# RandallBalestriero/noise-robust-vit

Hardware: AMD Instinct MI355X
Metric: images/sec (fwd+bwd+optimizer) ViT-B/16 224px bf16 (higher is better)
Workload: dtype bf16

## Files before the change

noise_robust_vit_amd/csrc/nrv_attn.hip:

```cpp
#include <type_traits>

#include "nrv_attn_common.hpp"

NRV_INTERNAL int nrv_attn_gen_supported(int B, int N, int H, int dh);
NRV_INTERNAL int nrv_attn_gen_fwd(const void* qkv, void* out, float* lse, int B, int N, int H, int dh, float scale, hipStream_t s);
NRV_INTERNAL int nrv_attn_gen_bwd(const void* qkv, const void* out, const void* dout, const float* lse, void* dqkv, float* delta_ws,
                     int B, int N, int H, int dh, float scale, hipStream_t s);
NRV_INTERNAL int nrv_attn_gen_probs(const void* qkv, const float* lse, float* probs, int B, int N, int H, int dh, float scale, hipStream_t s);

namespace {

using namespace nrv_attn;
struct AttnParams {
    const bf16_t* qkv;
    const bf16_t* out;
    const bf16_t* dout;
    bf16_t* o;
    bf16_t* dqkv;
    float* lse;
    float* delta;
    int B, N, H;
    float scale;
    long long q_rs, q_ws, q_hs, q_bs, o_rs, o_hs, o_bs;
};

void set_layout(AttnParams& p, int layout, int dh) {
    const long long T = (long long)p.B * p.N;
    if (layout & NRV_ATTN_QKV_BLOCKED) { p.q_rs = dh; p.q_ws = (long long)p.H * T * dh; p.q_hs = T * dh; p.q_bs = (long long)p.N * dh; }
    else { p.q_rs = 3ll * p.H * dh; p.q_ws = (long long)p.H * dh; p.q_hs = dh; p.q_bs = p.N * p.q_rs; }
    if (layout & NRV_ATTN_OUT_BLOCKED) { p.o_rs = dh; p.o_hs = T * dh; p.o_bs = (long long)p.N * dh; }
    else { p.o_rs = (long long)p.H * dh; p.o_hs = dh; p.o_bs = p.N * p.o_rs; }
}

template <int NT>
constexpr int atf_waves() { return NT <= 2 ? 1 : NT <= 4 ? 2 : 4; }

template <int NT>
__global__ __launch_bounds__(64 * atf_waves<NT>(), NT <= 13 ? 3 : 2) void attn_fwd_fat_kernel(const AttnParams p) {
    extern __shared__ __attribute__((aligned(16))) char smem[];
    constexpr int NP = NT * 16;
    constexpr int IMG = NP * 128;
    constexpr int NS = (NT + 1) / 2;
    constexpr int NJ = 2 * NP / 8;
    constexpr int ATF_WAVES = atf_waves<NT>();
    constexpr int JPW = NJ / ATF_WAVES;
    constexpr int MT = (NT == 13 || NT == 14) ? 1 : 2;
    const int tid = threadIdx.x, lane = tid & 63, wave = tid >> 6;
    const int N = p.N, H = p.H;
    const long long ldq = p.q_rs;
    const int b = blockIdx.x / H, h = blockIdx.x - b * H;
    const bf16_t* hb = p.qkv + (long long)b * p.q_bs + h * p.q_hs;
    const int g = lane >> 4, qc = lane & 15;
    const float sc = p.scale * LOG2E;
    const char* kimg = smem;
    const char* vimg = smem + IMG;

    const int npairs = (N + 31) >> 5;
    bf16x8_t qf[2][2];
    auto load_q = [&](int pair) {
#pragma unroll
        for (int t = 0; t < 2; ++t) {
            const int q = pair * 32 + t * 16 + qc;
            const int qr = q < N ? q : N - 1;
#pragma unroll
            for (int ks = 0; ks < 2; ++ks) qf[t][ks] = load_frag_global(hb + (long long)qr * ldq + ks * 32 + g * 8);
        }
    };
    if (wave < npairs) load_q(wave);
    {
        const __amdgpu_buffer_rsrc_t rk = make_rsrc(hb + p.q_ws, 0x7fffffffull), rv = make_rsrc(hb + 2 * p.q_ws, 0x7fffffffull);
        const int wave_u = __builtin_amdgcn_readfirstlane(wave);
#pragma unroll
        for (int i = 0; i < JPW; ++i) {
            const int j = wave_u * JPW + i;
            const bool isv = j >= NP / 8;
            const int r = 8 * (isv ? j - NP / 8 : j) + (lane >> 3);
            const int pos = lane & 7;
            const int c = isv ? ((((pos >> 1) ^ ((r >> 1) & 3)) << 1) | (pos & 1)) : (pos ^ ((r >> 1) & 7));
            const unsigned vo = (r < N) ? (unsigned)(r * ldq * 2 + c * 16) : NRV_OOB;
            if (isv) dma16_nt(rv, smem + j * 1024, vo);
            else dma16_nt(rk, smem + j * 1024, vo);
        }
    }
    __builtin_amdgcn_s_waitcnt(0x0F70);
    asm volatile("" ::: "memory");
    __syncthreads();

    const bf16x4_t zero4 = {0, 0, 0, 0};
    auto v_frag = [&](int kk, int dt) {
        const int q = (lane & 15) >> 2, pp = lane & 3;
        const int r0 = kk * 32 + 4 * g + q;
        const bf16x4_t lo = lds_read_tr16_b64(vimg + r0 * 128 + ((dt ^ ((r0 >> 1) & 3)) << 5) + pp * 8);
        if (2 * kk + 1 >= NT) return cat4(lo, zero4);
        return cat4(lo, lds_read_tr16_b64(vimg + (r0 + 16) * 128 + ((dt ^ (((r0 + 16) >> 1) & 3)) << 5) + pp * 8));
    };
    const int d_lane = (g & 1) ? 16 + 4 * (g - 1) : 4 * g;
    for (int pair = wave; pair < npairs; pair += ATF_WAVES) {
        f32x4_t st[2][NT];
        constexpr int KD = NT < 4 ? NT : 4;
        bf16x8_t kf[KD][2];
#pragma unroll
        for (int j = 0; j < KD - 1; ++j)
#pragma unroll
            for (int ks = 0; ks < 2; ++ks) kf[j][ks] = row_frag_img(kimg, j * 16, ks, lane);
#pragma unroll
        for (int kt = 0; kt < NT; ++kt) {
            if (kt + KD - 1 < NT) {
#pragma unroll
                for (int ks = 0; ks < 2; ++ks) kf[(kt + KD - 1) % KD][ks] = row_frag_img(kimg, (kt + KD - 1) * 16, ks, lane);
            }
#pragma unroll
            for (int t = 0; t < 2; ++t) {
                f32x4_t a = {0.f, 0.f, 0.f, 0.f};
#pragma unroll
                for (int ks = 0; ks < 2; ++ks) a = mfma16(kf[kt % KD][ks], qf[t][ks], a);
                st[t][kt] = a;
            }
        }
        __builtin_amdgcn_sched_barrier(0);
        const int q0 = pair * 32 + qc;
        if (pair + ATF_WAVES < npairs) load_q(pair + ATF_WAVES);
        bf16x8_t vf[2][4];
#pragma unroll
        for (int dt = 0; dt < 4; ++dt) vf[0][dt] = v_frag(0, dt);
        float m[2], l[2];
        bf16x8_t pf[2][NS];
#pragma unroll
        for (int t = 0; t < 2; ++t) {
            float mm = -INFINITY;
#pragma unroll
            for (int kt = 0; kt < NT; ++kt) {
#pragma unroll
                for (int e = 0; e < 4; ++e) {
                    if (kt >= NT - MT) mm = fmaxf(mm, (kt * 16 + 4 * g + e < N) ? st[t][kt][e] : -INFINITY);
                    else mm = fmaxf(mm, st[t][kt][e]);
                }
            }
            mm = fmaxf(mm, __shfl_xor(mm, 16, 64));
            mm = fmaxf(mm, __shfl_xor(mm, 32, 64));
            mm *= sc;
            float ll = 0.f;
#pragma unroll
            for (int kt = 0; kt < NT; ++kt) {
#pragma unroll
                for (int e = 0; e < 4; ++e) {
                    float pv = __builtin_amdgcn_exp2f(fmaf(st[t][kt][e], sc, -mm));
                    if (kt >= NT - MT) pv = (kt * 16 + 4 * g + e < N) ? pv : 0.f;
                    st[t][kt][e] = pv;
                    ll += pv;
                }
                if (kt & 1) pf[t][kt >> 1] = pack_frag(st[t][kt - 1], st[t][kt]);
                else if (kt == NT - 1) pf[t][kt >> 1] = pack_frag(st[t][kt], f32x4_t{0.f, 0.f, 0.f, 0.f});
            }
            ll += __shfl_xor(ll, 16, 64);
            ll += __shfl_xor(ll, 32, 64);
            m[t] = mm;
            l[t] = ll;
        }
        __builtin_amdgcn_sched_barrier(0);
        f32x4_t o[2][4];
#pragma unroll
        for (int t = 0; t < 2; ++t)
#pragma unroll
            for (int dt = 0; dt < 4; ++dt) o[t][dt] = f32x4_t{0.f, 0.f, 0.f, 0.f};
#pragma unroll
        for (int kk = 0; kk < NS; ++kk) {
            if (kk + 1 < NS) {
#pragma unroll
                for (int dt = 0; dt < 4; ++dt) vf[(kk + 1) & 1][dt] = v_frag(kk + 1, dt);
            }
#pragma unroll
            for (int dt = 0; dt < 4; ++dt)
#pragma unroll
                for (int t = 0; t < 2; ++t) o[t][dt] = mfma16(vf[kk & 1][dt], pf[t][kk], o[t][dt]);
        }
        __builtin_amdgcn_sched_barrier(0);
#pragma unroll
        for (int t = 0; t < 2; ++t) {
            const int q = q0 + t * 16;
            const float inv = 1.0f / l[t];
            u32x4_t ov[2];
#pragma unroll
            for (int pr = 0; pr < 2; ++pr) {
                const f32x4_t oa = o[t][2 * pr] * inv, ob = o[t][2 * pr + 1] * inv;
                const auto lo = __builtin_amdgcn_permlane16_swap(pack_bf16x2(oa[0], oa[1]), pack_bf16x2(ob[0], ob[1]), false, false);
                const auto hi = __builtin_amdgcn_permlane16_swap(pack_bf16x2(oa[2], oa[3]), pack_bf16x2(ob[2], ob[3]), false, false);
                ov[pr] = u32x4_t{lo[0], hi[0], lo[1], hi[1]};
            }
            if (q < N) {
                bf16_t* dst = p.o + (long long)b * p.o_bs + h * p.o_hs + (long long)q * p.o_rs + d_lane;
#pragma unroll
                for (int pr = 0; pr < 2; ++pr) *reinterpret_cast<u32x4_t*>(dst + 32 * pr) = ov[pr];
                if (g == 0) p.lse[((long long)b * H + h) * N + q] = (m[t] + __builtin_amdgcn_logf(l[t])) * LN2;
            }
        }
    }
}

__device__ __forceinline__ bf16x8_t row_frag_bwd(const char* img, int rb, int ks, int lane) {
    return lds_read_b128(img + vimg_off(rb + (lane & 15), ks * 4 + (lane >> 4)));
}

__device__ __forceinline__ void store_tile_bf16(bf16_t* row_ptr , const f32x4_t (&acc)[4],
                                                float mul, int g, bool ok) {
    const int d_lane = (g & 1) ? 16 + 4 * (g - 1) : 4 * g;
#pragma unroll
    for (int pr = 0; pr < 2; ++pr) {
        const f32x4_t a = acc[2 * pr] * mul, b = acc[2 * pr + 1] * mul;
        const auto lo = __builtin_amdgcn_permlane16_swap(pack_bf16x2(a[0], a[1]), pack_bf16x2(b[0], b[1]), false, false);
        const auto hi = __builtin_amdgcn_permlane16_swap(pack_bf16x2(a[2], a[3]), pack_bf16x2(b[2], b[3]), false, false);
        if (ok) *reinterpret_cast<u32x4_t*>(row_ptr + 32 * pr + d_lane) = u32x4_t{lo[0], hi[0], lo[1], hi[1]};
    }
}

template <int NT>
__device__ __forceinline__ void dma_two_images(char* smem, const bf16_t* src0, long long ld0, const bf16_t* src1, long long ld1,
                                               int N, int wave, int lane) {
    constexpr int NP = NT * 16;
    constexpr int PW = 4 * NT / atf_waves<NT>();
    const __amdgpu_buffer_rsrc_t r0 = make_rsrc(src0, 0x7fffffffull), r1 = make_rsrc(src1, 0x7fffffffull);
    const int wave_u = __builtin_amdgcn_readfirstlane(wave);
#pragma unroll
    for (int i = 0; i < PW; ++i) {
        const int j = wave_u * PW + i;
        const bool second = j >= NP / 8;
        const int r = 8 * (second ? j - NP / 8 : j) + (lane >> 3);
        const int pos = lane & 7;
        const int c = (((pos >> 1) ^ ((r >> 1) & 3)) << 1) | (pos & 1);
        const unsigned vo = (r < N) ? (unsigned)(r * (second ? ld1 : ld0) * 2 + c * 16) : NRV_OOB;
        if (second) dma16(r1, smem + j * 1024, vo);
        else dma16(r0, smem + j * 1024, vo);
    }
}

template <int NT>
__global__ __launch_bounds__(64 * atf_waves<NT>(), NT <= 13 ? 3 : 2) void attn_bwd_dq_fat_kernel(const AttnParams p) {
    extern __shared__ __attribute__((aligned(16))) char smem[];
    constexpr int ATF_WAVES = atf_waves<NT>();
    constexpr int NP = NT * 16;
    constexpr int NS = (NT + 1) / 2;
    constexpr int MT = (NT == 13 || NT == 14) ? 1 : 2;
    const char* kimg = smem;
    const char* vimg = smem + NP * 128;
    const int tid = threadIdx.x, lane = tid & 63, wave = tid >> 6;
    const int N = p.N, H = p.H;
    const int b = blockIdx.x / H, h = blockIdx.x - b * H;
    const long long ldq = p.q_rs, ldo = p.o_rs;
    const bf16_t* qbase = p.qkv + (long long)b * p.q_bs + h * p.q_hs;
    const bf16_t* obase = p.out + (long long)b * p.o_bs + h * p.o_hs;
    const bf16_t* dobase = p.dout + (long long)b * p.o_bs + h * p.o_hs;
    const int g = lane >> 4, qc = lane & 15;
    const float sc = p.scale * LOG2E;
    const int npairs = (N + 31) >> 5;

    bf16x8_t qf[2][2], dof[2][2];
    float dl[2], lse2[2];
    auto load_rows = [&](int pair) {
#pragma unroll
        for (int t = 0; t < 2; ++t) {
            const int q = pair * 32 + t * 16 + qc;
            const int qr = q < N ? q : N - 1;
            float d = 0.f;
#pragma unroll
            for (int ks = 0; ks < 2; ++ks) {
                qf[t][ks] = load_frag_global(qbase + (long long)qr * ldq + ks * 32 + g * 8);
                dof[t][ks] = load_frag_global(dobase + (long long)qr * ldo + ks * 32 + g * 8);
                const bf16x8_t of = load_frag_global(obase + (long long)qr * ldo + ks * 32 + g * 8);
#pragma unroll
                for (int e = 0; e < 8; ++e) d += bf16_to_f32((unsigned short)dof[t][ks][e]) * bf16_to_f32((unsigned short)of[e]);
            }
            d += __shfl_xor(d, 16, 64);
            d += __shfl_xor(d, 32, 64);
            dl[t] = d;
            const long long sidx = ((long long)b * H + h) * N + qr;
            lse2[t] = p.lse[sidx] * LOG2E;
            if (g == 0 && q < N) p.delta[sidx] = d;
        }
    };
    if (wave < npairs) load_rows(wave);
    dma_two_images<NT>(smem, qbase + p.q_ws, ldq, qbase + 2 * p.q_ws, ldq, N, wave, lane);
    __builtin_amdgcn_s_waitcnt(0x0F70);
    asm volatile("" ::: "memory");
    __syncthreads();

    const bf16x4_t zero4 = {0, 0, 0, 0};
    for (int pair = wave; pair < npairs; pair += ATF_WAVES) {
        f32x4_t dq[2][4];
#pragma unroll
        for (int t = 0; t < 2; ++t)
#pragma unroll
            for (int dt = 0; dt < 4; ++dt) dq[t][dt] = f32x4_t{0.f, 0.f, 0.f, 0.f};
        auto step = [&](const int kk, auto last_c) {
            constexpr bool LAST = decltype(last_c)::value;
            f32x4_t ds[2][2];
#pragma unroll
            for (int hf = 0; hf < 2; ++hf) {
                const int kt = 2 * kk + hf;
                if (!LAST || hf == 0 || (NT % 2 == 0)) {
                    bf16x8_t kr[2], vr[2];
#pragma unroll
                    for (int ks = 0; ks < 2; ++ks) {
                        kr[ks] = row_frag_bwd(kimg, kt * 16, ks, lane);
                        vr[ks] = row_frag_bwd(vimg, kt * 16, ks, lane);
                    }
#pragma unroll
                    for (int t = 0; t < 2; ++t) {
                        f32x4_t st = {0.f, 0.f, 0.f, 0.f}, dp = {0.f, 0.f, 0.f, 0.f};
#pragma unroll
                        for (int ks = 0; ks < 2; ++ks) {
                            st = mfma16(kr[ks], qf[t][ks], st);
                            dp = mfma16(vr[ks], dof[t][ks], dp);
                        }
#pragma unroll
                        for (int e = 0; e < 4; ++e) {
                            float pv = __builtin_amdgcn_exp2f(fmaf(st[e], sc, -lse2[t]));
                            if (LAST) pv = (kt * 16 + 4 * g + e < N) ? pv : 0.f;
                            ds[t][hf][e] = pv * (dp[e] - dl[t]);
                        }
                    }
                } else {
#pragma unroll
                    for (int t = 0; t < 2; ++t) ds[t][hf] = f32x4_t{0.f, 0.f, 0.f, 0.f};
                }
            }
            bf16x8_t dsf[2];
#pragma unroll
            for (int t = 0; t < 2; ++t) dsf[t] = pack_frag(ds[t][0], ds[t][1]);
#pragma unroll
            for (int dt = 0; dt < 4; ++dt) {
                const int q4 = (lane & 15) >> 2, pp = lane & 3;
                const int r0 = kk * 32 + 4 * g + q4;
                const int c = 2 * dt + (pp >> 1);
                const bf16x4_t lo = lds_read_tr16_b64(kimg + vimg_off(r0, c) + (pp & 1) * 8);
                const bf16x4_t hi = (!LAST || NT % 2 == 0) ? lds_read_tr16_b64(kimg + vimg_off(r0 + 16, c) + (pp & 1) * 8) : zero4;
                const bf16x8_t ktr = cat4(lo, hi);
#pragma unroll
                for (int t = 0; t < 2; ++t) dq[t][dt] = mfma16(ktr, dsf[t], dq[t][dt]);
            }
        };
#pragma unroll 1
        for (int kk = 0; kk < NS - 1; ++kk) step(kk, std::false_type{});
        step(NS - 1, std::true_type{});
        const int q0 = pair * 32 + qc;
        f32x4_t keep[2][4];
#pragma unroll
        for (int t = 0; t < 2; ++t)
#pragma unroll
            for (int dt = 0; dt < 4; ++dt) keep[t][dt] = dq[t][dt];
        if (pair + ATF_WAVES < npairs) load_rows(pair + ATF_WAVES);
#pragma unroll
        for (int t = 0; t < 2; ++t) {
            const int q = q0 + t * 16;
            store_tile_bf16(p.dqkv + (long long)b * p.q_bs + h * p.q_hs + (long long)(q < N ? q : 0) * ldq, keep[t], p.scale, g, q < N);
        }
    }
}

template <int NT>
__global__ __launch_bounds__(64 * atf_waves<NT>(), 2) void attn_bwd_dkv_fat_kernel(const AttnParams p) {
    extern __shared__ __attribute__((aligned(16))) char smem[];
    constexpr int ATF_WAVES = atf_waves<NT>(), ATF_THREADS = 64 * ATF_WAVES;
    constexpr int NP = NT * 16;
    constexpr int NS = (NT + 1) / 2;
    constexpr int NPS = NS * 32;
    const char* qimg = smem;
    const char* doimg = smem + NP * 128;
    float* lse2s = reinterpret_cast<float*>(smem + 2 * NP * 128);
    float* dels = lse2s + NPS;
    const int tid = threadIdx.x, lane = tid & 63, wave = tid >> 6;
    const int N = p.N, H = p.H;
    const int b = blockIdx.x / H, h = blockIdx.x - b * H;
    const long long ldq = p.q_rs, ldo = p.o_rs;
    const bf16_t* qbase = p.qkv + (long long)b * p.q_bs + h * p.q_hs;
    const bf16_t* dobase = p.dout + (long long)b * p.o_bs + h * p.o_hs;
    const int g = lane >> 4, kc = lane & 15;
    const float sc = p.scale * LOG2E;
    const int npairs = (N + 31) >> 5;

    bf16x8_t kf[2][2], vf[2][2];
    auto load_rows = [&](int pair) {
#pragma unroll
        for (int t = 0; t < 2; ++t) {
            const int key = pair * 32 + t * 16 + kc;
            const int kr = key < N ? key : N - 1;
#pragma unroll
            for (int ks = 0; ks < 2; ++ks) {
                kf[t][ks] = load_frag_global(qbase + p.q_ws + (long long)kr * ldq + ks * 32 + g * 8);
                vf[t][ks] = load_frag_global(qbase + 2 * p.q_ws + (long long)kr * ldq + ks * 32 + g * 8);
            }
        }
    };
    if (wave < npairs) load_rows(wave);
    for (int i = tid; i < NPS; i += ATF_THREADS) {
        const long long sidx = ((long long)b * H + h) * N + i;
        lse2s[i] = i < N ? p.lse[sidx] * LOG2E : INFINITY;
        dels[i] = i < N ? p.delta[sidx] : 0.f;
    }
    dma_two_images<NT>(smem, qbase, ldq, dobase, ldo, N, wave, lane);
    __builtin_amdgcn_s_waitcnt(0x0F70);
    asm volatile("" ::: "memory");
    __syncthreads();

    const bf16x4_t zero4 = {0, 0, 0, 0};
    auto tr_frag = [&](const char* img, int qq, int dt, auto last_c) {
        const int q4 = (lane & 15) >> 2, pp = lane & 3;
        const int r0 = qq * 32 + 4 * g + q4;
        const int c = 2 * dt + (pp >> 1);
        const bf16x4_t lo = lds_read_tr16_b64(img + vimg_off(r0, c) + (pp & 1) * 8);
        const bf16x4_t hi = (!decltype(last_c)::value || NT % 2 == 0) ? lds_read_tr16_b64(img + vimg_off(r0 + 16, c) + (pp & 1) * 8) : zero4;
        return cat4(lo, hi);
    };
    for (int pair = wave; pair < npairs; pair += ATF_WAVES) {
        f32x4_t dk[2][4], dv[2][4];
#pragma unroll
        for (int t = 0; t < 2; ++t)
#pragma unroll
            for (int dt = 0; dt < 4; ++dt) {
                dk[t][dt] = f32x4_t{0.f, 0.f, 0.f, 0.f};
                dv[t][dt] = dk[t][dt];
            }
        auto step = [&](const int qq, auto last_c) {
            constexpr bool LAST = decltype(last_c)::value;
            f32x4_t pt[2][2], ds[2][2];
#pragma unroll
            for (int hf = 0; hf < 2; ++hf) {
                const int qt = 2 * qq + hf;
                if (!LAST || hf == 0 || (NT % 2 == 0)) {
                    bf16x8_t qr[2], dor[2];
#pragma unroll
                    for (int ks = 0; ks < 2; ++ks) {
                        qr[ks] = row_frag_bwd(qimg, qt * 16, ks, lane);
                        dor[ks] = row_frag_bwd(doimg, qt * 16, ks, lane);
                    }
                    const f32x4_t l4 = *reinterpret_cast<const f32x4_t*>(lse2s + qt * 16 + 4 * g);
                    const f32x4_t d4 = *reinterpret_cast<const f32x4_t*>(dels + qt * 16 + 4 * g);
#pragma unroll
                    for (int t = 0; t < 2; ++t) {
                        f32x4_t st = {0.f, 0.f, 0.f, 0.f}, dp = {0.f, 0.f, 0.f, 0.f};
#pragma unroll
                        for (int ks = 0; ks < 2; ++ks) {
                            st = mfma16(qr[ks], kf[t][ks], st);
                            dp = mfma16(dor[ks], vf[t][ks], dp);
                        }
#pragma unroll
                        for (int e = 0; e < 4; ++e) {
                            const float pv = __builtin_amdgcn_exp2f(fmaf(st[e], sc, -l4[e]));
                            pt[t][hf][e] = pv;
                            ds[t][hf][e] = pv * (dp[e] - d4[e]);
                        }
                    }
                } else {
#pragma unroll
                    for (int t = 0; t < 2; ++t) {
                        pt[t][hf] = f32x4_t{0.f, 0.f, 0.f, 0.f};
                        ds[t][hf] = pt[t][hf];
                    }
                }
            }
            bf16x8_t pf[2], dsf[2];
#pragma unroll
            for (int t = 0; t < 2; ++t) {
                pf[t] = pack_frag(pt[t][0], pt[t][1]);
                dsf[t] = pack_frag(ds[t][0], ds[t][1]);
            }
#pragma unroll
            for (int dt = 0; dt < 4; ++dt) {
                const bf16x8_t dotr = tr_frag(doimg, qq, dt, last_c);
                const bf16x8_t qtr = tr_frag(qimg, qq, dt, last_c);
#pragma unroll
                for (int t = 0; t < 2; ++t) {
                    dv[t][dt] = mfma16(dotr, pf[t], dv[t][dt]);
                    dk[t][dt] = mfma16(qtr, dsf[t], dk[t][dt]);
                }
            }
        };
#pragma unroll 1
        for (int qq = 0; qq < NS - 1; ++qq) step(qq, std::false_type{});
        step(NS - 1, std::true_type{});
        const int k0 = pair * 32 + kc;
        if (pair + ATF_WAVES < npairs) load_rows(pair + ATF_WAVES);
#pragma unroll
        for (int t = 0; t < 2; ++t) {
            const int key = k0 + t * 16;
            bf16_t* row = p.dqkv + (long long)b * p.q_bs + h * p.q_hs + (long long)(key < N ? key : 0) * ldq;
            store_tile_bf16(row + p.q_ws, dk[t], p.scale, g, key < N);
            store_tile_bf16(row + 2 * p.q_ws, dv[t], 1.0f, g, key < N);
        }
    }
}

template <int NT>
int launch_fwd_fat_nt(const AttnParams& p, hipStream_t s) {
    constexpr int lds = 2 * NT * 16 * 128;
    static int attr = (int)hipFuncSetAttribute(reinterpret_cast<const void*>(attn_fwd_fat_kernel<NT>),
                                               hipFuncAttributeMaxDynamicSharedMemorySize, lds);
    if (attr != 0) return attr;
    hipLaunchKernelGGL((attn_fwd_fat_kernel<NT>), dim3(p.B * p.H), dim3(64 * atf_waves<NT>()), lds, s, p);
    NRV_CHECK_LAUNCH();
    return 0;
}

int launch_fwd_fat(const AttnParams& p, hipStream_t s) {
    const int nt = (p.N + 15) / 16;
    if (nt <= 2) return launch_fwd_fat_nt<2>(p, s);
    if (nt <= 4) return launch_fwd_fat_nt<4>(p, s);
    if (nt <= 6) return launch_fwd_fat_nt<6>(p, s);
    if (nt <= 8) return launch_fwd_fat_nt<8>(p, s);
    if (nt <= 10) return launch_fwd_fat_nt<10>(p, s);
    if (nt <= 12) return launch_fwd_fat_nt<12>(p, s);
    if (nt == 13) return launch_fwd_fat_nt<13>(p, s);
    if (nt == 14) return launch_fwd_fat_nt<14>(p, s);
    return launch_fwd_fat_nt<16>(p, s);
}

template <int NT>
int launch_bwd_fat_nt(const AttnParams& p, hipStream_t s) {
    constexpr int lds_dq = 2 * NT * 16 * 128;
    constexpr int lds_dkv = 2 * NT * 16 * 128 + 2 * ((NT + 1) / 2) * 32 * 4;
    static int a1 = (int)hipFuncSetAttribute(reinterpret_cast<const void*>(attn_bwd_dq_fat_kernel<NT>),
                                             hipFuncAttributeMaxDynamicSharedMemorySize, lds_dq);
    static int a2 = (int)hipFuncSetAttribute(reinterpret_cast<const void*>(attn_bwd_dkv_fat_kernel<NT>),
                                             hipFuncAttributeMaxDynamicSharedMemorySize, lds_dkv);
    if (a1 != 0) return a1;
    if (a2 != 0) return a2;
    hipLaunchKernelGGL((attn_bwd_dq_fat_kernel<NT>), dim3(p.B * p.H), dim3(64 * atf_waves<NT>()), lds_dq, s, p);
    NRV_CHECK_LAUNCH();
    hipLaunchKernelGGL((attn_bwd_dkv_fat_kernel<NT>), dim3(p.B * p.H), dim3(64 * atf_waves<NT>()), lds_dkv, s, p);
    NRV_CHECK_LAUNCH();
    return 0;
}

int launch_bwd_fat(const AttnParams& p, hipStream_t s) {
    const int nt = (p.N + 15) / 16;
    if (nt <= 2) return launch_bwd_fat_nt<2>(p, s);
    if (nt <= 4) return launch_bwd_fat_nt<4>(p, s);
    if (nt <= 6) return launch_bwd_fat_nt<6>(p, s);
    if (nt <= 8) return launch_bwd_fat_nt<8>(p, s);
    if (nt <= 10) return launch_bwd_fat_nt<10>(p, s);
    if (nt <= 12) return launch_bwd_fat_nt<12>(p, s);
    if (nt == 13) return launch_bwd_fat_nt<13>(p, s);
    if (nt == 14) return launch_bwd_fat_nt<14>(p, s);
    return launch_bwd_fat_nt<16>(p, s);
}

__global__ __launch_bounds__(256) void attn_probs_kernel(const AttnParams p, float* __restrict__ probs) {
    __shared__ float qs[16][DH + 1];
    const bf16_t* __restrict__ qkv = p.qkv;
    const float* __restrict__ lse = p.lse;
    const int N = p.N, H = p.H;
    const float scale = p.scale;
    const int bh = blockIdx.x, q0 = blockIdx.y * 16;
    const int b = bh / H, h = bh - b * H;
    const long long ldq = p.q_rs;
    const bf16_t* base = qkv + (long long)b * p.q_bs + h * p.q_hs;
    for (int i = threadIdx.x; i < 16 * DH; i += 256) {
        const int r = i / DH, d = i - r * DH;
        qs[r][d] = (q0 + r < N) ? bf16_to_f32(base[(long long)(q0 + r) * ldq + d]) : 0.f;
    }
    __syncthreads();
    const int qi = threadIdx.x & 15;
    const int q = q0 + qi;
    const float l = q < N ? lse[((long long)b * H + h) * N + q] : 0.f;
    for (int key = threadIdx.x >> 4; key < N; key += 16) {
        const bf16_t* kp = base + p.q_ws + (long long)key * ldq;
        float acc = 0.f;
#pragma unroll
        for (int c = 0; c < DH / 8; ++c) {
            const bf16x8_t kv = load_frag_global(kp + c * 8);
#pragma unroll
            for (int e = 0; e < 8; ++e) acc = fmaf(qs[qi][c * 8 + e], bf16_to_f32((unsigned short)kv[e]), acc);
        }
        if (q < N) probs[(((long long)b * H + h) * N + q) * N + key] = __expf(acc * scale - l);
    }
}

int shape_class(int B, int N, int H, int dh) {
    if (B <= 0 || N <= 0 || H <= 0) return 0;
    if (dh == DH && N <= 256) return (long long)B * H > 0x7fffffffll ? 0 : 1;
    return nrv_attn_gen_supported(B, N, H, dh) ? 2 : 0;
}

}

static bool layout_ok(int layout, int cls, int B, int N, int H, int dh) {
    if (layout & ~(NRV_ATTN_QKV_BLOCKED | NRV_ATTN_OUT_BLOCKED)) return false;
    if (layout != 0 && cls != 1) return false;
    return 2ll * 3 * H * (long long)B * N * dh < 0x7fffffffll;
}

extern "C" int nrv_attn_fwd(const void* qkv_bf16, void* out_bf16, float* lse,
                            int B, int N, int H, int dh, float scale, int layout, void* stream) {
    if (!qkv_bf16 || !out_bf16 || !lse) return NRV_ERR_NULL;
    const int cls = shape_class(B, N, H, dh);
    if (cls == 0 || !layout_ok(layout, cls, B, N, H, dh)) return NRV_ERR_SHAPE;
    if (!nrv_aligned16(qkv_bf16) || !nrv_aligned16(out_bf16)) return NRV_ERR_ALIGN;
    if (cls == 2) return nrv_attn_gen_fwd(qkv_bf16, out_bf16, lse, B, N, H, dh, scale, static_cast<hipStream_t>(stream));
    AttnParams p{};
    p.qkv = static_cast<const bf16_t*>(qkv_bf16);
    p.o = static_cast<bf16_t*>(out_bf16);
    p.lse = lse;
    p.B = B; p.N = N; p.H = H; p.scale = scale;
    set_layout(p, layout, dh);
    hipStream_t s = static_cast<hipStream_t>(stream);
    return launch_fwd_fat(p, s);
}

extern "C" int nrv_attn_bwd(const void* qkv_bf16, const void* out_bf16, const void* dout_bf16, const float* lse,
                            void* dqkv_bf16, float* delta_ws,
                            int B, int N, int H, int dh, float scale, int layout, void* stream) {
    if (!qkv_bf16 || !out_bf16 || !dout_bf16 || !lse || !dqkv_bf16 || !delta_ws) return NRV_ERR_NULL;
    const int cls = shape_class(B, N, H, dh);
    if (cls == 0 || !layout_ok(layout, cls, B, N, H, dh)) return NRV_ERR_SHAPE;
    if (!nrv_aligned16(qkv_bf16) || !nrv_aligned16(out_bf16) || !nrv_aligned16(dout_bf16) || !nrv_aligned16(dqkv_bf16))
        return NRV_ERR_ALIGN;
    if (cls == 2)
        return nrv_attn_gen_bwd(qkv_bf16, out_bf16, dout_bf16, lse, dqkv_bf16, delta_ws, B, N, H, dh, scale, static_cast<hipStream_t>(stream));
    AttnParams p{};
    p.qkv = static_cast<const bf16_t*>(qkv_bf16);
    p.out = static_cast<const bf16_t*>(out_bf16);
    p.dout = static_cast<const bf16_t*>(dout_bf16);
    p.dqkv = static_cast<bf16_t*>(dqkv_bf16);
    p.lse = const_cast<float*>(lse);
    p.delta = delta_ws;
    p.B = B; p.N = N; p.H = H; p.scale = scale;
    set_layout(p, layout, dh);
    hipStream_t s = static_cast<hipStream_t>(stream);
    return launch_bwd_fat(p, s);
}

extern "C" int nrv_attn_probs(const void* qkv_bf16, const float* lse, float* probs,
                              int B, int N, int H, int dh, float scale, int layout, void* stream) {
    if (!qkv_bf16 || !lse || !probs) return NRV_ERR_NULL;
    const int cls = shape_class(B, N, H, dh);
    if (cls == 0 || !layout_ok(layout, cls, B, N, H, dh)) return NRV_ERR_SHAPE;
    if (!nrv_aligned16(qkv_bf16)) return NRV_ERR_ALIGN;
    hipStream_t s = static_cast<hipStream_t>(stream);
    if (cls == 2) return nrv_attn_gen_probs(qkv_bf16, lse, probs, B, N, H, dh, scale, s);
    AttnParams p{};
    p.qkv = static_cast<const bf16_t*>(qkv_bf16);
    p.lse = const_cast<float*>(lse);
    p.B = B; p.N = N; p.H = H; p.scale = scale;
    set_layout(p, layout, dh);
    hipLaunchKernelGGL(attn_probs_kernel, dim3((unsigned)(B * H), (unsigned)((N + 15) / 16)), dim3(256), 0, s, p, probs);
    NRV_CHECK_LAUNCH();
    return 0;
}
```

Measured before the change: 7901.

## Overlap K/V LDS image DMA with first-tile compute and restructure dQ kernel

Splits the K and V LDS image DMA so each wave issues interleaved rows, then waits only for the K image (partial vmcnt) before starting QK^T, deferring the V wait and barrier to just before P·V. Q/dO/lse prefetches use volatile asm loads so they are not reordered behind the barrier. The dQ backward kernel now processes one 16-row tile at a time, computes delta from P·dP instead of reading the forward output O, and prefetches the next tile's rows. This aims to cut startup latency and register pressure, but relies on hand-encoded waitcnt values and an extra barrier per kernel, which is fragile if the DMA issue order differs from what the counters assume.

```diff
diff --git a/noise_robust_vit_amd/csrc/nrv_attn.hip b/noise_robust_vit_amd/csrc/nrv_attn.hip
--- a/noise_robust_vit_amd/csrc/nrv_attn.hip
+++ b/noise_robust_vit_amd/csrc/nrv_attn.hip
@@ -35,56 +35,93 @@
 template <int NT>
 constexpr int atf_waves() { return NT <= 2 ? 1 : NT <= 4 ? 2 : 4; }
 
+template <int VM>
+__device__ __forceinline__ void wait_vm_and_barrier() {
+    static_assert(VM >= 0 && VM < 64, "vmcnt is a 6-bit counter");
+    __builtin_amdgcn_sched_barrier(0);
+    __builtin_amdgcn_s_waitcnt(0x0070 | (VM & 15) | ((VM >> 4) << 14));
+    asm volatile("" ::: "memory");
+    __builtin_amdgcn_s_barrier();
+    asm volatile("" ::: "memory");
+    __builtin_amdgcn_sched_barrier(0);
+}
+
+__device__ __forceinline__ bf16x8_t load_frag_global_early(const bf16_t* p) {
+    bf16x8_t r;
+    asm volatile("global_load_dwordx4 %0, %1, off" : "=v"(r) : "v"(p) : "memory");
+    return r;
+}
+__device__ __forceinline__ float load_f32_global_early(const float* p) {
+    float r;
+    asm volatile("global_load_dword %0, %1, off" : "=v"(r) : "v"(p) : "memory");
+    return r;
+}
+template <typename T>
+__device__ __forceinline__ void frag_landed(T& x) { asm volatile("" : "+v"(x)); }
+__device__ __forceinline__ void next_rows_landed() { __builtin_amdgcn_s_waitcnt(0x0F70); }
+
+template <int NT>
+constexpr int IMG_DMA_MIN = 2 * NT / atf_waves<NT>();
+template <int NT, bool PAIR, bool NONTEMPORAL>
+__device__ __forceinline__ void dma_image(char* img, const bf16_t* src, long long ld, int N, int wave_u, int lane) {
+    constexpr int NR = 2 * NT, W = atf_waves<NT>();
+    const __amdgpu_buffer_rsrc_t rs = make_rsrc(src, 0x7fffffffull);
+#pragma unroll
+    for (int i = 0; i < (NR + W - 1) / W; ++i) {
+        const int j = i * W + wave_u;
+        if ((i + 1) * W <= NR || j < NR) {
+            const int r = 8 * j + (lane >> 3);
+            const int pos = lane & 7;
+            const int c = PAIR ? ((((pos >> 1) ^ ((r >> 1) & 3)) << 1) | (pos & 1)) : (pos ^ ((r >> 1) & 7));
+            const unsigned vo = (r < N) ? (unsigned)(r * ld * 2 + c * 16) : NRV_OOB;
+            if (NONTEMPORAL) dma16_nt(rs, img + j * 1024, vo);
+            else dma16(rs, img + j * 1024, vo);
+        }
+    }
+}
+
 template <int NT>
 __global__ __launch_bounds__(64 * atf_waves<NT>(), NT <= 13 ? 3 : 2) void attn_fwd_fat_kernel(const AttnParams p) {
     extern __shared__ __attribute__((aligned(16))) char smem[];
     constexpr int NP = NT * 16;
     constexpr int IMG = NP * 128;
     constexpr int NS = (NT + 1) / 2;
-    constexpr int NJ = 2 * NP / 8;
     constexpr int ATF_WAVES = atf_waves<NT>();
-    constexpr int JPW = NJ / ATF_WAVES;
     constexpr int MT = (NT == 13 || NT == 14) ? 1 : 2;
-    const int tid = threadIdx.x, lane = tid & 63, wave = tid >> 6;
+    const int tid = threadIdx.x, lane = tid & 63;
+    const int wave = __builtin_amdgcn_readfirstlane(tid >> 6);
     const int N = p.N, H = p.H;
     const long long ldq = p.q_rs;
     const int b = blockIdx.x / H, h = blockIdx.x - b * H;
     const bf16_t* hb = p.qkv + (long long)b * p.q_bs + h * p.q_hs;
     const int g = lane >> 4, qc = lane & 15;
     const float sc = p.scale * LOG2E;
-    const char* kimg = smem;
-    const char* vimg = smem + IMG;
+    char* kimg = smem;
+    char* vimg = smem + IMG;
 
     const int npairs = (N + 31) >> 5;
     bf16x8_t qf[2][2];
-    auto load_q = [&](int pair) {
+    auto load_q = [&](int pair, auto early_c) {
 #pragma unroll
         for (int t = 0; t < 2; ++t) {
             const int q = pair * 32 + t * 16 + qc;
             const int qr = q < N ? q : N - 1;
 #pragma unroll
-            for (int ks = 0; ks < 2; ++ks) qf[t][ks] = load_frag_global(hb + (long long)qr * ldq + ks * 32 + g * 8);
+            for (int ks = 0; ks < 2; ++ks) {
+                const bf16_t* src = hb + (long long)qr * ldq + ks * 32 + g * 8;
+                if (decltype(early_c)::value) qf[t][ks] = load_frag_global_early(src);
+                else qf[t][ks] = load_frag_global(src);
+            }
         }
     };
-    if (wave < npairs) load_q(wave);
-    {
-        const __amdgpu_buffer_rsrc_t rk = make_rsrc(hb + p.q_ws, 0x7fffffffull), rv = make_rsrc(hb + 2 * p.q_ws, 0x7fffffffull);
-        const int wave_u = __builtin_amdgcn_readfirstlane(wave);
-#pragma unroll
-        for (int i = 0; i < JPW; ++i) {
-            const int j = wave_u * JPW + i;
-            const bool isv = j >= NP / 8;
-            const int r = 8 * (isv ? j - NP / 8 : j) + (lane >> 3);
-            const int pos = lane & 7;
-            const int c = isv ? ((((pos >> 1) ^ ((r >> 1) & 3)) << 1) | (pos & 1)) : (pos ^ ((r >> 1) & 7));
-            const unsigned vo = (r < N) ? (unsigned)(r * ldq * 2 + c * 16) : NRV_OOB;
-            if (isv) dma16_nt(rv, smem + j * 1024, vo);
-            else dma16_nt(rk, smem + j * 1024, vo);
-        }
-    }
-    __builtin_amdgcn_s_waitcnt(0x0F70);
-    asm volatile("" ::: "memory");
-    __syncthreads();
+    if (wave < npairs) load_q(wave, std::true_type{});
+    dma_image<NT, false, true>(kimg, hb + p.q_ws, ldq, N, wave, lane);
+    dma_image<NT, true, true>(vimg, hb + 2 * p.q_ws, ldq, N, wave, lane);
+    wait_vm_and_barrier<IMG_DMA_MIN<NT>>();
+#pragma unroll
+    for (int t = 0; t < 2; ++t)
+#pragma unroll
+        for (int ks = 0; ks < 2; ++ks) frag_landed(qf[t][ks]);
 
     const bf16x4_t zero4 = {0, 0, 0, 0};
     auto v_frag = [&](int kk, int dt) {
@@ -118,8 +155,9 @@
             }
         }
         __builtin_amdgcn_sched_barrier(0);
+        if (pair == wave) wait_vm_and_barrier<0>();
         const int q0 = pair * 32 + qc;
-        if (pair + ATF_WAVES < npairs) load_q(pair + ATF_WAVES);
+        if (pair + ATF_WAVES < npairs) load_q(pair + ATF_WAVES, std::false_type{});
         bf16x8_t vf[2][4];
 #pragma unroll
         for (int dt = 0; dt < 4; ++dt) vf[0][dt] = v_frag(0, dt);
@@ -175,6 +213,7 @@
                 for (int t = 0; t < 2; ++t) o[t][dt] = mfma16(vf[kk & 1][dt], pf[t][kk], o[t][dt]);
         }
         __builtin_amdgcn_sched_barrier(0);
+        next_rows_landed();
 #pragma unroll
         for (int t = 0; t < 2; ++t) {
             const int q = q0 + t * 16;
@@ -195,6 +234,7 @@
             }
         }
     }
+    if (wave >= npairs) wait_vm_and_barrier<0>();
 }
 
 __device__ __forceinline__ bf16x8_t row_frag_bwd(const char* img, int rb, int ks, int lane) {
@@ -210,26 +250,6 @@
         const auto lo = __builtin_amdgcn_permlane16_swap(pack_bf16x2(a[0], a[1]), pack_bf16x2(b[0], b[1]), false, false);
         const auto hi = __builtin_amdgcn_permlane16_swap(pack_bf16x2(a[2], a[3]), pack_bf16x2(b[2], b[3]), false, false);
         if (ok) *reinterpret_cast<u32x4_t*>(row_ptr + 32 * pr + d_lane) = u32x4_t{lo[0], hi[0], lo[1], hi[1]};
-    }
-}
-
-template <int NT>
-__device__ __forceinline__ void dma_two_images(char* smem, const bf16_t* src0, long long ld0, const bf16_t* src1, long long ld1,
-                                               int N, int wave, int lane) {
-    constexpr int NP = NT * 16;
-    constexpr int PW = 4 * NT / atf_waves<NT>();
-    const __amdgpu_buffer_rsrc_t r0 = make_rsrc(src0, 0x7fffffffull), r1 = make_rsrc(src1, 0x7fffffffull);
-    const int wave_u = __builtin_amdgcn_readfirstlane(wave);
-#pragma unroll
-    for (int i = 0; i < PW; ++i) {
-        const int j = wave_u * PW + i;
-        const bool second = j >= NP / 8;
-        const int r = 8 * (second ? j - NP / 8 : j) + (lane >> 3);
-        const int pos = lane & 7;
-        const int c = (((pos >> 1) ^ ((r >> 1) & 3)) << 1) | (pos & 1);
-        const unsigned vo = (r < N) ? (unsigned)(r * (second ? ld1 : ld0) * 2 + c * 16) : NRV_OOB;
-        if (second) dma16(r1, smem + j * 1024, vo);
-        else dma16(r0, smem + j * 1024, vo);
     }
 }
 
@@ -240,120 +260,120 @@
     constexpr int NP = NT * 16;
     constexpr int NS = (NT + 1) / 2;
     constexpr int MT = (NT == 13 || NT == 14) ? 1 : 2;
-    const char* kimg = smem;
-    const char* vimg = smem + NP * 128;
-    const int tid = threadIdx.x, lane = tid & 63, wave = tid >> 6;
+    char* kimg = smem;
+    char* vimg = smem + NP * 128;
+    const int tid = threadIdx.x, lane = tid & 63;
+    const int wave = __builtin_amdgcn_readfirstlane(tid >> 6);
     const int N = p.N, H = p.H;
     const int b = blockIdx.x / H, h = blockIdx.x - b * H;
     const long long ldq = p.q_rs, ldo = p.o_rs;
     const bf16_t* qbase = p.qkv + (long long)b * p.q_bs + h * p.q_hs;
-    const bf16_t* obase = p.out + (long long)b * p.o_bs + h * p.o_hs;
     const bf16_t* dobase = p.dout + (long long)b * p.o_bs + h * p.o_hs;
     const int g = lane >> 4, qc = lane & 15;
     const float sc = p.scale * LOG2E;
     const int npairs = (N + 31) >> 5;
 
-    bf16x8_t qf[2][2], dof[2][2];
-    float dl[2], lse2[2];
-    auto load_rows = [&](int pair) {
+    bf16x8_t qf[2], dof[2];
+    float lsev;
+    auto load_rows = [&](int tile, auto early_c) {
+        constexpr bool EARLY = decltype(early_c)::value;
+        const int q = tile * 16 + qc;
+        const int qr = q < N ? q : N - 1;
+#pragma unroll
+        for (int ks = 0; ks < 2; ++ks) {
+            const bf16_t* qs = qbase + (long long)qr * ldq + ks * 32 + g * 8;
+            const bf16_t* ds = dobase + (long long)qr * ldo + ks * 32 + g * 8;
+            qf[ks] = EARLY ? load_frag_global_early(qs) : load_frag_global(qs);
+            dof[ks] = EARLY ? load_frag_global_early(ds) : load_frag_global(ds);
+        }
+        const float* ls = p.lse + ((long long)b * H + h) * N + qr;
+        lsev = EARLY ? load_f32_global_early(ls) : *ls;
+    };
+    if (wave < npairs) load_rows(2 * wave, std::true_type{});
+    dma_image<NT, true, false>(kimg, qbase + p.q_ws, ldq, N, wave, lane);
+    dma_image<NT, true, false>(vimg, qbase + 2 * p.q_ws, ldq, N, wave, lane);
+    wait_vm_and_barrier<IMG_DMA_MIN<NT>>();
+#pragma unroll
+    for (int ks = 0; ks < 2; ++ks) {
+        frag_landed(qf[ks]);
+        frag_landed(dof[ks]);
+    }
+    frag_landed(lsev);
+
+    const bf16x4_t zero4 = {0, 0, 0, 0};
+    for (int pair = wave; pair < npairs; pair += ATF_WAVES) {
+        const int q0 = pair * 32 + qc;
 #pragma unroll
         for (int t = 0; t < 2; ++t) {
-            const int q = pair * 32 + t * 16 + qc;
-            const int qr = q < N ? q : N - 1;
+            if (t == 1 && pair * 32 + 16 >= N) break;
+            int ln = lane;
+            asm volatile("" : "+v"(ln));
+            const float nl = -lsev * LOG2E;
+            f32x4_t pr[NT], dp[NT];
+#pragma unroll
+            for (int kt = 0; kt < NT; ++kt) {
+                f32x4_t st = {0.f, 0.f, 0.f, 0.f};
+#pragma unroll
+                for (int ks = 0; ks < 2; ++ks) st = mfma16(row_frag_bwd(kimg, kt * 16, ks, ln), qf[ks], st);
+#pragma unroll
+                for (int e = 0; e < 4; ++e) {
+                    float pv = __builtin_amdgcn_exp2f(fmaf(st[e], sc, nl));
+                    if (kt >= NT - MT) pv = (kt * 16 + 4 * g + e < N) ? pv : 0.f;
+                    pr[kt][e] = pv;
+                }
+            }
+            __builtin_amdgcn_sched_barrier(0);
+            if (t == 0 && pair == wave) wait_vm_and_barrier<0>();
             float d = 0.f;
 #pragma unroll
-            for (int ks = 0; ks < 2; ++ks) {
-                qf[t][ks] = load_frag_global(qbase + (long long)qr * ldq + ks * 32 + g * 8);
-                dof[t][ks] = load_frag_global(dobase + (long long)qr * ldo + ks * 32 + g * 8);
-                const bf16x8_t of = load_frag_global(obase + (long long)qr * ldo + ks * 32 + g * 8);
-#pragma unroll
-                for (int e = 0; e < 8; ++e) d += bf16_to_f32((unsigned short)dof[t][ks][e]) * bf16_to_f32((unsigned short)of[e]);
-            }
+            for (int kt = 0; kt < NT; ++kt) {
+                f32x4_t a = {0.f, 0.f, 0.f, 0.f};
+#pragma unroll
+                for (int ks = 0; ks < 2; ++ks) a = mfma16(row_frag_bwd(vimg, kt * 16, ks, ln), dof[ks], a);
+                dp[kt] = a;
+#pragma unroll
+                for (int e = 0; e < 4; ++e) d = fmaf(pr[kt][e], a[e], d);
+            }
+            __builtin_amdgcn_sched_barrier(0);
             d += __shfl_xor(d, 16, 64);
             d += __shfl_xor(d, 32, 64);
-            dl[t] = d;
-            const long long sidx = ((long long)b * H + h) * N + qr;
-            lse2[t] = p.lse[sidx] * LOG2E;
-            if (g == 0 && q < N) p.delta[sidx] = d;
-        }
-    };
-    if (wave < npairs) load_rows(wave);
-    dma_two_images<NT>(smem, qbase + p.q_ws, ldq, qbase + 2 * p.q_ws, ldq, N, wave, lane);
-    __builtin_amdgcn_s_waitcnt(0x0F70);
-    asm volatile("" ::: "memory");
-    __syncthreads();
-
-    const bf16x4_t zero4 = {0, 0, 0, 0};
-    for (int pair = wave; pair < npairs; pair += ATF_WAVES) {
-        f32x4_t dq[2][4];
-#pragma unroll
-        for (int t = 0; t < 2; ++t)
-#pragma unroll
-            for (int dt = 0; dt < 4; ++dt) dq[t][dt] = f32x4_t{0.f, 0.f, 0.f, 0.f};
-        auto step = [&](const int kk, auto last_c) {
-            constexpr bool LAST = decltype(last_c)::value;
-            f32x4_t ds[2][2];
-#pragma unroll
-            for (int hf = 0; hf < 2; ++hf) {
-                const int kt = 2 * kk + hf;
-                if (!LAST || hf == 0 || (NT % 2 == 0)) {
-                    bf16x8_t kr[2], vr[2];
-#pragma unroll
-                    for (int ks = 0; ks < 2; ++ks) {
-                        kr[ks] = row_frag_bwd(kimg, kt * 16, ks, lane);
-                        vr[ks] = row_frag_bwd(vimg, kt * 16, ks, lane);
-                    }
-#pragma unroll
-                    for (int t = 0; t < 2; ++t) {
-                        f32x4_t st = {0.f, 0.f, 0.f, 0.f}, dp = {0.f, 0.f, 0.f, 0.f};
-#pragma unroll
-                        for (int ks = 0; ks < 2; ++ks) {
-                            st = mfma16(kr[ks], qf[t][ks], st);
-                            dp = mfma16(vr[ks], dof[t][ks], dp);
-                        }
-#pragma unroll
-                        for (int e = 0; e < 4; ++e) {
-                            float pv = __builtin_amdgcn_exp2f(fmaf(st[e], sc, -lse2[t]));
-                            if (LAST) pv = (kt * 16 + 4 * g + e < N) ? pv : 0.f;
-                            ds[t][hf][e] = pv * (dp[e] - dl[t]);
-                        }
-                    }
-                } else {
-#pragma unroll
-                    for (int t = 0; t < 2; ++t) ds[t][hf] = f32x4_t{0.f, 0.f, 0.f, 0.f};
+            const int q = q0 + t * 16;
+            if (g == 0 && q < N) p.delta[((long long)b * H + h) * N + q] = d;
+            bf16x8_t dsf[NS];
+#pragma unroll
+            for (int kt = 0; kt < NT; ++kt) {
+#pragma unroll
+                for (int e = 0; e < 4; ++e) dp[kt][e] = pr[kt][e] * (dp[kt][e] - d);
+                if (kt & 1) dsf[kt >> 1] = pack_frag(dp[kt - 1], dp[kt]);
+                else if (kt == NT - 1) dsf[kt >> 1] = pack_frag(dp[kt], f32x4_t{0.f, 0.f, 0.f, 0.f});
+            }
+            __builtin_amdgcn_sched_barrier(0);
+            if (t == 0) {
+                if (pair * 32 + 16 < N) load_rows(2 * pair + 1, std::false_type{});
+                else if (pair + ATF_WAVES < npairs) load_rows(2 * (pair + ATF_WAVES), std::false_type{});
+            } else if (pair + ATF_WAVES < npairs) load_rows(2 * (pair + ATF_WAVES), std::false_type{});
+            f32x4_t dq[4];
+#pragma unroll
+            for (int dt = 0; dt < 4; ++dt) dq[dt] = f32x4_t{0.f, 0.f, 0.f, 0.f};
+            asm volatile("" : "+v"(ln));
+#pragma unroll
+            for (int kk = 0; kk < NS; ++kk) {
+#pragma unroll
+                for (int dt = 0; dt < 4; ++dt) {
+                    const int q4 = (ln & 15) >> 2, pp = ln & 3;
+                    const int r0 = kk * 32 + 4 * (ln >> 4) + q4;
+                    const int c = 2 * dt + (pp >> 1);
+                    const bf16x4_t lo = lds_read_tr16_b64(kimg + vimg_off(r0, c) + (pp & 1) * 8);
+                    const bf16x4_t hi = (2 * kk + 1 < NT) ? lds_read_tr16_b64(kimg + vimg_off(r0 + 16, c) + (pp & 1) * 8) : zero4;
+                    dq[dt] = mfma16(cat4(lo, hi), dsf[kk], dq[dt]);
                 }
             }
-            bf16x8_t dsf[2];
-#pragma unroll
-            for (int t = 0; t < 2; ++t) dsf[t] = pack_frag(ds[t][0], ds[t][1]);
-#pragma unroll
-            for (int dt = 0; dt < 4; ++dt) {
-                const int q4 = (lane & 15) >> 2, pp = lane & 3;
-                const int r0 = kk * 32 + 4 * g + q4;
-                const int c = 2 * dt + (pp >> 1);
-                const bf16x4_t lo = lds_read_tr16_b64(kimg + vimg_off(r0, c) + (pp & 1) * 8);
-                const bf16x4_t hi = (!LAST || NT % 2 == 0) ? lds_read_tr16_b64(kimg + vimg_off(r0 + 16, c) + (pp & 1) * 8) : zero4;
-                const bf16x8_t ktr = cat4(lo, hi);
-#pragma unroll
-                for (int t = 0; t < 2; ++t) dq[t][dt] = mfma16(ktr, dsf[t], dq[t][dt]);
-            }
-        };
-#pragma unroll 1
-        for (int kk = 0; kk < NS - 1; ++kk) step(kk, std::false_type{});
-        step(NS - 1, std::true_type{});
-        const int q0 = pair * 32 + qc;
-        f32x4_t keep[2][4];
-#pragma unroll
-        for (int t = 0; t < 2; ++t)
-#pragma unroll
-            for (int dt = 0; dt < 4; ++dt) keep[t][dt] = dq[t][dt];
-        if (pair + ATF_WAVES < npairs) load_rows(pair + ATF_WAVES);
-#pragma unroll
-        for (int t = 0; t < 2; ++t) {
-            const int q = q0 + t * 16;
-            store_tile_bf16(p.dqkv + (long long)b * p.q_bs + h * p.q_hs + (long long)(q < N ? q : 0) * ldq, keep[t], p.scale, g, q < N);
-        }
-    }
+            next_rows_landed();
+            store_tile_bf16(p.dqkv + (long long)b * p.q_bs + h * p.q_hs + (long long)(q < N ? q : 0) * ldq, dq, p.scale, g, q < N);
+            __builtin_amdgcn_sched_barrier(0);
+        }
+    }
+    if (wave >= npairs) wait_vm_and_barrier<0>();
 }
 
 template <int NT>
@@ -396,7 +416,11 @@
         lse2s[i] = i < N ? p.lse[sidx] * LOG2E : INFINITY;
         dels[i] = i < N ? p.delta[sidx] : 0.f;
     }
-    dma_two_images<NT>(smem, qbase, ldq, dobase, ldo, N, wave, lane);
+    {
+        const int wave_u = __builtin_amdgcn_readfirstlane(wave);
+        dma_image<NT, true, false>(smem, qbase, ldq, N, wave_u, lane);
+        dma_image<NT, true, false>(smem + NP * 128, dobase, ldo, N, wave_u, lane);
+    }
     __builtin_amdgcn_s_waitcnt(0x0F70);
     asm volatile("" ::: "memory");
     __syncthreads();
```

New measurement: 7941 (median of 6 runs). No clear change (+0.5%).
